# fenghansen/YOND_public

Measured on AMD Instinct MI355X. Metric: Bayer megapixels/sec end-to-end (NLE+VST+denoise+iVST), higher is better.
Workload: dtype f32 (3x3 convolutions: f32 operands as two f16 halves -- 22-23 significant bits -- on the f16 MFMA, 3 products per f32 product, f32 accumulate; per-layer error vs float64 asserted <= 2x the f32 direct kernel's and <= 2e-5 of max|ref| (tests/test_hip_conv.py; measured 1.3e-6 vs 1.5e-6), whole frame v

## Files before the change

### yond_public_amd/csrc/conv_s2_tall.hip

```cpp
#include "common.h"

typedef _Float16 f16x8 __attribute__((ext_vector_type(8)));
typedef _Float16 f16x4 __attribute__((ext_vector_type(4)));
#define S2T_GLOBAL __attribute__((address_space(1)))

namespace {
constexpr int S2T_TH = 8;
constexpr int S2T_IH = (S2T_TH - 1) * 2 + 3;
constexpr int S2T_IW = 31 * 2 + 3;
constexpr int S2T_HALF = (S2T_IW + 1) / 2;
constexpr int S2T_TWP = 2 * S2T_HALF;
constexpr int S2T_PLANE = S2T_IH * S2T_TWP * 4;
constexpr int S2T_IMG = 4 * S2T_PLANE + 4;
constexpr int S2T_W = 9 * 2 * 2 * 64 * 4;
constexpr int S2T_NWV = S2T_W / 4;
constexpr int S2T_NWT = (S2T_NWV + 511) / 512;
constexpr int S2T_NITEM = S2T_IH * S2T_IW * 4;
constexpr int S2T_NIN = (S2T_NITEM + 511) / 512;
constexpr int S2T_FILM = 1536;
constexpr int S2T_W_OFF = S2T_IMG, S2T_FILM_OFF = S2T_W_OFF + 2 * S2T_W;
constexpr int S2T_SMEM = (S2T_FILM_OFF + 2 * S2T_FILM) * 4;
static_assert(S2T_SMEM <= 160 * 1024, "LDS budget");
static_assert((S2T_NIN - 1) * 512 < S2T_NITEM, "only a thread's last item may lie past the tile");

__device__ __forceinline__ float s2t_silu(float x) {
    return x * __builtin_amdgcn_rcpf(1.0f + __builtin_amdgcn_exp2f(x * -1.44269504088896341f));
}
}

template <bool D2>
__global__ __launch_bounds__(512) void conv_s2_tall_kernel(const YondConvDesc d) {
    extern __shared__ __attribute__((aligned(16))) float smem[];
    const int tid = threadIdx.x, lane = tid & 63, wave = __builtin_amdgcn_readfirstlane(tid >> 6);
    const int li = lane & 31, lh = lane >> 5;
    const int rg = wave & 3, cg = wave >> 2;
    const int nct = d.Cout / 64, ntx = (d.Wo + 31) / 32, nty = (d.Ho + S2T_TH - 1) / S2T_TH;
    const int total = nct * ntx * nty * d.N;
    const int G = gridDim.x;
    const int lslot = (G % 8 == 0) ? (blockIdx.x % 8) * (G / 8) + blockIdx.x / 8 : blockIdx.x;
    const int nchunk = d.C0 / 16;
    const bool rev = d.tile_order != 0;
    const int PS0 = YOND_SP_PLANE_UNITS(d.H, d.W);
    if (lslot >= total) return;
    const bool clk_on = d.clk != nullptr && blockIdx.x == 0 && tid == 0;
    unsigned long long clk_c0 = 0, clk_r0 = 0;
    if (clk_on) { clk_c0 = __builtin_amdgcn_s_memtime(); clk_r0 = __builtin_amdgcn_s_memrealtime(); }
    asm volatile("" : "+v"(clk_c0), "+v"(clk_r0));
    float* dst_v = d.dst;
    char* dst2_v = (char*)d.dst2;
    unsigned int* word_v = d.status;
    unsigned long long* clk_v = d.clk;
    asm volatile("" : "+v"(dst_v), "+v"(dst2_v), "+v"(word_v), "+v"(clk_v));
    int nct_v = nct, ntx_v = ntx, nty_v = nty;
    unsigned ps2_v = (unsigned)YOND_SP_PLANE_UNITS(d.Ho, d.Wo);
    asm volatile("" : "+v"(nct_v), "+v"(ntx_v), "+v"(nty_v), "+v"(ps2_v));

    {
        const int nf = (d.ebatch ? d.N : 1) * d.Cout;
        for (int i = tid; i < nf; i += 512) {
            smem[S2T_FILM_OFF + i] = d.escale ? d.escale[i] : 1.0f;
            smem[S2T_FILM_OFF + S2T_FILM + i] = d.eshift ? d.eshift[i] : 0.0f;
        }
    }

    int in_lds[S2T_NIN];
#pragma unroll
    for (int k = 0; k < S2T_NIN; ++k) {
        const int it = tid + k * 512;
        const int pix = it >> 2, py = pix / S2T_IW, px = pix % S2T_IW;
        const int lp = py * S2T_TWP + (px & 1) * S2T_HALF + (px >> 1);
        in_lds[k] = it < S2T_NITEM ? (it & 3) * S2T_PLANE + lp * 4 : 4 * S2T_PLANE;
    }

    struct Tile { int ct, n, ox0, oy0; };
    auto origin = [&](int t) {
        Tile T;
        int b = t;
        T.ct = b % nct_v; b /= nct_v;
        const int tx = b % ntx_v; b /= ntx_v;
        const int ty = b % nty_v, n = b / nty_v;
        T.n = __builtin_amdgcn_readfirstlane(rev ? d.N - 1 - n : n);
        T.ct = __builtin_amdgcn_readfirstlane(T.ct);
        T.ox0 = __builtin_amdgcn_readfirstlane((rev ? ntx_v - 1 - tx : tx) * 32);
        T.oy0 = __builtin_amdgcn_readfirstlane((rev ? nty_v - 1 - ty : ty) * S2T_TH);
        return T;
    };
    unsigned voff[S2T_NIN];
    auto decode = [&](const Tile& T) {
#pragma unroll
        for (int k = 0; k < S2T_NIN; ++k) {
            const int it = tid + k * 512;
            const int pix = it >> 2, py = pix / S2T_IW, px = pix % S2T_IW;
            const int gy = T.oy0 * 2 - 1 + py, gx = T.ox0 * 2 - 1 + px;
            const bool in = it < S2T_NITEM && gy >= 0 && gy < d.H && gx >= 0 && gx < d.W;
            voff[k] = ((unsigned)(it & 3) * (unsigned)PS0 + (unsigned)(in ? gy * d.W + gx : d.H * d.W)) * 16u;
        }
    };
    auto uniform_ptr = [&](const void* p) {
        const unsigned long long a = (unsigned long long)(uintptr_t)p;
        const unsigned lo = __builtin_amdgcn_readfirstlane((unsigned)a), hi = __builtin_amdgcn_readfirstlane((unsigned)(a >> 32));
        return (const char*)(uintptr_t)(((unsigned long long)hi << 32) | lo);
    };
    auto in_base = [&](const Tile& T, int ch) { return (const char*)d.src0 + (size_t)(T.n * nchunk + ch) * 4 * (size_t)PS0 * 16; };
    auto w_base = [&](const Tile& T, int ch) { return uniform_ptr(d.wpk + ((size_t)T.ct * nchunk + ch) * S2T_W); };
    f32x4 vin[S2T_NIN];
    auto issue_load = [&](auto kc, const char* ib) __attribute__((always_inline)) {
        constexpr int k = decltype(kc)::value;
        vin[k] = *(const S2T_GLOBAL f32x4*)(const S2T_GLOBAL char*)(ib + voff[k]);
    };
    auto issue_dma = [&](auto kc, const char* wsrc, float* wbuf) __attribute__((always_inline)) {
        constexpr int k = decltype(kc)::value;
        const unsigned lds0 = (unsigned)(uintptr_t)(__attribute__((address_space(3))) float*)wbuf;
        const int it = tid + k * 512;
        const int it_wave = __builtin_amdgcn_readfirstlane(it - lane);
        const unsigned lds_wave = __builtin_amdgcn_readfirstlane(lds0 + (unsigned)it_wave * 16u);
        const unsigned vo = (unsigned)it * 16u;
        if ((k + 1) * 512 <= S2T_NWV || it_wave < S2T_NWV)
            asm volatile("s_mov_b32 m0, %0\n\ts_nop 0\n\tglobal_load_lds_dwordx4 %1, %2" ::"s"(lds_wave), "v"(vo), "s"(wsrc) : "memory");
    };
    auto write_in = [&]() __attribute__((always_inline)) {
#pragma unroll
        for (int k = 0; k < S2T_NIN; ++k) *(f32x4*)(smem + in_lds[k]) = vin[k];
    };

    f32x16 acc[2][2];
    auto zero_acc = [&]() {
#pragma unroll
        for (int a = 0; a < 2; ++a)
#pragma unroll
            for (int m = 0; m < 2; ++m)
#pragma unroll
                for (int r = 0; r < 16; ++r) acc[a][m][r] = 0.0f;
    };

    const int x_off = (lh * 2) * S2T_PLANE + ((rg * 4) * S2T_TWP + li) * 4;
    const int w_off = ((lh * 2) * 64 + cg * 32 + li) * 4;
    const bool wave_hi = wave >= 4;
    const char* ib_s = nullptr;
    const char* wsrc_s = nullptr;
    auto mfma_step = [&](const float* wcur, float* wnext, auto&& prep) __attribute__((always_inline)) {
        typedef const __attribute__((address_space(3))) f16x8* lds_h8;
        const __attribute__((address_space(3))) float* xb = (const __attribute__((address_space(3))) float*)(smem + x_off);
        const __attribute__((address_space(3))) float* wb = (const __attribute__((address_space(3))) float*)(wcur + w_off);
        constexpr int R = 5, NQ = 3 * R, XD = 3, Q0 = 2, NQW = NQ - Q0, NOPS = S2T_NWT + S2T_NIN;
        f16x8 xr[XD][2], wt[2][3][2];
        auto loadX = [&](auto qc) __attribute__((always_inline)) {
            constexpr int q = decltype(qc)::value, dx = q / R, r = q % R;
            constexpr int xo = (dx & 1) * S2T_HALF + (dx >> 1);
#pragma unroll
            for (int p = 0; p < 2; ++p) xr[q % XD][p] = *(lds_h8)(xb + p * S2T_PLANE + (r * S2T_TWP + xo) * 4);
        };
        auto loadW = [&](auto dc) __attribute__((always_inline)) {
            constexpr int dx = decltype(dc)::value;
#pragma unroll
            for (int dy = 0; dy < 3; ++dy)
#pragma unroll
                for (int p = 0; p < 2; ++p) wt[dx % 2][dy][p] = *(lds_h8)(wb + (((dy * 3 + dx) * 4 + p) * 64) * 4);
        };
        loadW(IntC<0>{});
        loadX(IntC<0>{});
        loadX(IntC<1>{});
        static_for<0, NQ>([&](auto qc) __attribute__((always_inline)) {
            constexpr int q = decltype(qc)::value, dx = q / R, r = q % R;
            constexpr bool wpre = r == 2 && dx < 2;
            if constexpr (q + 2 < NQ) loadX(IntC<q + 2>{});
            if constexpr (wpre) loadW(IntC<dx + 1>{});
            constexpr int nmf = 3 * ((r <= 2 ? 1 : 0) + (r >= 2 ? 1 : 0));
#pragma unroll
            for (int a = 0; a < 3; ++a) {
#pragma unroll
                for (int m = 0; m < 2; ++m) {
                    const int dy = r - 2 * m;
                    if (dy < 0 || dy > 2) continue;
                    acc[a == 1 ? 0 : 1][m] = __builtin_amdgcn_mfma_f32_32x32x16_f16(wt[dx % 2][dy][a == 2 ? 1 : 0], xr[q % XD][a == 0 ? 1 : 0],
                                                                                    acc[a == 1 ? 0 : 1][m], 0, 0, 0);
                }
            }
            if constexpr (q == 0) { if (wave_hi) __builtin_amdgcn_s_setprio(1); }
            if constexpr (q == NQ / 2) { if (wave_hi) __builtin_amdgcn_s_setprio(0); }
            if constexpr (q == Q0 - 1) prep();
            constexpr int qq = q >= Q0 ? q - Q0 : 0;
            constexpr int o_lo = q >= Q0 ? (qq * NOPS + NQW - 1) / NQW : 0, o_hi = q >= Q0 ? ((qq + 1) * NOPS + NQW - 1) / NQW : 0;
            static_for<o_lo, (o_hi < NOPS ? o_hi : NOPS)>([&](auto oc) __attribute__((always_inline)) {
                constexpr int o = decltype(oc)::value;
                if constexpr (o < S2T_NWT) issue_dma(IntC<o>{}, wsrc_s, wnext);
                else issue_load(IntC<o - S2T_NWT>{}, ib_s);
            });
            constexpr int nrd = (q + 2 < NQ ? 2 : 0) + (wpre ? 6 : 0);
            constexpr int l_lo = o_lo > S2T_NWT ? o_lo : S2T_NWT, nld = o_hi > l_lo ? o_hi - l_lo : 0;
            if constexpr (nrd > 0) __builtin_amdgcn_sched_group_barrier(0x100, nrd, 0);
#pragma unroll
            for (int i = 0; i < nmf; ++i) {
                __builtin_amdgcn_sched_group_barrier(0x008, 1, 0);
                if (i == 0 && nld > 0) __builtin_amdgcn_sched_group_barrier(0x020, nld, 0);
            }
        });
    };

    float slope_eff = d.post_act == 2 ? d.slope : 1.0f;
    asm volatile("" : "+v"(slope_eff));
    YondRange amax;
    auto epilogue = [&](const Tile& T) __attribute__((always_inline)) {
        const int ox = T.ox0 + li;
        const bool col_ok = ox < d.Wo;
        const int cbase = T.ct * 64 + cg * 32 + 4 * lh;
        const float* fs = smem + S2T_FILM_OFF + (d.ebatch ? T.n * d.Cout : 0) + cbase;
        const long long hw = (long long)d.Ho * d.Wo;
        f32x4 es[4], et[4];
#pragma unroll
        for (int g = 0; g < 4; ++g) {
            es[g] = *(const f32x4*)(fs + 8 * g);
            et[g] = *(const f32x4*)(fs + S2T_FILM + 8 * g);
        }
#pragma unroll
        for (int m = 0; m < 2; ++m) {
            const int oy = T.oy0 + rg * 2 + m;
            const bool ok = col_ok && oy < d.Ho;
            const long long pixo = (long long)oy * d.Wo + ox;
            float* op = dst_v + (((long long)T.n * (d.Cout / 4) + cbase / 4) * hw + pixo) * 4;
            const long long gstep = 8LL * hw;
#pragma unroll
            for (int g = 0; g < 4; ++g) {
                f32x4 v;
#pragma unroll
                for (int e = 0; e < 4; ++e) {
                    float x = acc[0][m][4 * g + e];
                    x = fmaf(acc[1][m][4 * g + e], 1.0f / 2048.0f, x);
                    x = fmaf(x, es[g][e], et[g][e]);
                    x = x > 0.0f ? x : x * slope_eff;
                    v[e] = x + 0.0f;
                }
                if (ok) *(S2T_GLOBAL f32x4*)(S2T_GLOBAL float*)(op + g * gstep) = v;
                if constexpr (D2) {
                    f32x4 a;
#pragma unroll
                    for (int e = 0; e < 4; ++e) a[e] = s2t_silu(v[e]);
                    amax.add(a);
                    const f16x4 h = {(_Float16)a[0], (_Float16)a[1], (_Float16)a[2], (_Float16)a[3]};
                    const int c8 = cbase - 4 * lh + 8 * g;
                    const size_t PS2 = (size_t)ps2_v;
                    char* pp = dst2_v + ((size_t)(((T.n * (d.Cout / 16) + (c8 >> 4)) * 2 + ((c8 >> 3) & 1)) * 2) * PS2 + (size_t)pixo) * 16 + lh * 8;
                    if (ok) *(S2T_GLOBAL f16x4*)(S2T_GLOBAL char*)pp = h;
                    const f16x4 l = {(_Float16)((a[0] - (float)h[0]) * 2048.0f), (_Float16)((a[1] - (float)h[1]) * 2048.0f),
                                     (_Float16)((a[2] - (float)h[2]) * 2048.0f), (_Float16)((a[3] - (float)h[3]) * 2048.0f)};
                    if (ok) *(S2T_GLOBAL f16x4*)(S2T_GLOBAL char*)(pp + PS2 * 16) = l;
                }
            }
        }
    };

    struct Cur { int tile, ch; };
    auto adv = [&](Cur c) {
        Cur n;
        const bool last = c.ch + 1 == nchunk;
        n.tile = last ? c.tile + G : c.tile;
        n.ch = last ? 0 : c.ch + 1;
        return n;
    };
    Cur cs = {lslot, 0};
    Tile lt = origin(lslot), cur = lt;
    auto park = [&](Tile& T) { asm volatile("" : "+v"(T.ct), "+v"(T.n), "+v"(T.ox0), "+v"(T.oy0)); };
    park(cur);
    float* w0 = smem + S2T_W_OFF;
    float* w1 = w0 + S2T_W;
    decode(lt);
    {
        const char* ws = w_base(lt, 0);
        const char* ib = in_base(lt, 0);
        static_for<0, S2T_NWT>([&](auto kc) __attribute__((always_inline)) { issue_dma(kc, ws, w0); });
        static_for<0, S2T_NIN>([&](auto kc) __attribute__((always_inline)) { issue_load(kc, ib); });
    }
    zero_acc();
    asm volatile("s_waitcnt vmcnt(0)" ::: "memory");
    write_in();
    asm volatile("s_waitcnt vmcnt(0) lgkmcnt(0)\n\ts_barrier" ::: "memory");
    while (true) {
        const bool last_ch = cs.ch + 1 == nchunk;
        const Cur cn = adv(cs);
        auto prep = [&]() __attribute__((always_inline)) {
            if (last_ch && cn.tile < total) {
                lt = origin(cn.tile);
                decode(lt);
            }
            ib_s = in_base(lt, cn.ch);
            wsrc_s = w_base(lt, cn.ch);
        };
        mfma_step(w0, w1, prep);
        asm volatile("s_waitcnt lgkmcnt(0)\n\ts_barrier" ::: "memory");
        asm volatile("s_waitcnt vmcnt(0)" ::: "memory");
        write_in();
        if (last_ch) {
            epilogue(cur);
            zero_acc();
            cur = lt;
            park(cur);
        }
        asm volatile("s_waitcnt lgkmcnt(0)\n\ts_barrier" ::: "memory");
        if (cn.tile >= total) break;
        cs = cn;
        float* t = w0;
        w0 = w1;
        w1 = t;
    }
    if constexpr (D2) {
        if (word_v && !amax.at_most(65504.0f)) atomicOr(word_v, YOND_STATUS_HALF_OVERFLOW);
    }
    if (clk_on) {
        atomicAdd(clk_v, __builtin_amdgcn_s_memtime() - clk_c0);
        atomicAdd(clk_v + 1, __builtin_amdgcn_s_memrealtime() - clk_r0);
    }
}

static bool s2t_takes(const YondConvDesc& d) {
    if (d.ksize != 3 || d.stride != 2 || d.shuffle != 0 || d.tn != 64 || !d.src0 || d.src1 || d.C1 != 0 || !d.dst || !d.wpk) return false;
    if (d.in_fmt != YOND_FMT_SPLIT_PLANES || d.out_fmt != YOND_FMT_PLANES4 || d.res_fmt || d.res || d.out4_dst || d.pre_act) return false;
    if (d.post_act != 0 && d.post_act != 2) return false;
    if (d.N <= 0 || d.H <= 0 || d.W <= 0 || d.Ho != (d.H + 1) / 2 || d.Wo != (d.W + 1) / 2) return false;
    if (d.C0 <= 0 || d.C0 % 16 || d.Cout <= 0 || d.Cout % 64) return false;
    if ((long long)(d.ebatch ? d.N : 1) * d.Cout > S2T_FILM) return false;
    if ((long long)d.N * d.H * d.W > 0x7fffffffLL) return false;
    if ((long long)d.N * (d.C0 / 16) * 4 * YOND_SP_PLANE_UNITS(d.H, d.W) * 4 >= 0x7fffffffLL) return false;
    if ((long long)YOND_SP_PLANE_UNITS(d.H, d.W) * 16 * 4 >= 0x7fffffffLL) return false;
    const long long tiles = (long long)(d.Cout / 64) * ((d.Wo + 31) / 32) * ((d.Ho + S2T_TH - 1) / S2T_TH) * d.N;
    if (tiles > 0x7fffffffLL) return false;
    if (d.Wo <= 16) {
        const int f = d.Wo <= 8 ? 4 : 2;
        const long long subs = (long long)d.N * ((d.Ho + 3) / 4) * ((d.Wo + 32 / f - 1) / (32 / f));
        const long long tiles_f = (long long)(d.Cout / 64) * ((subs + f - 1) / f), tiles4 = (long long)(d.Cout / 64) * ((d.Ho + 3) / 4) * d.N;
        const bool fits = (long long)d.H * d.W * d.C0 * 4 * f < (1LL << 31);
        if (fits && (tiles_f + 255) / 256 < (tiles4 + 255) / 256) return false;
    }
    return true;
}

extern "C" int yond_conv_s2_tall_supported(const YondConvDesc* d) { return (d && (d->algo == 3 || d->algo == 7) && s2t_takes(*d)) ? 1 : 0; }

template <bool D2>
static int launch_s2t(const YondConvDesc& d, hipStream_t st) {
    static bool attr_set = false;
    auto kern = conv_s2_tall_kernel<D2>;
    if (!attr_set) {
        hipError_t e = hipFuncSetAttribute((const void*)kern, hipFuncAttributeMaxDynamicSharedMemorySize, S2T_SMEM);
        if (e != hipSuccess) return (int)e;
        attr_set = true;
    }
    const long long total = (long long)(d.Cout / 64) * ((d.Wo + 31) / 32) * ((d.Ho + S2T_TH - 1) / S2T_TH) * d.N;
    const int grid = total < 256 ? (int)total : 256;
    hipLaunchKernelGGL(kern, dim3(grid), dim3(512), S2T_SMEM, st, d);
    YOND_LAUNCH_CHECK();
    return YOND_OK;
}

int yond_conv_s2_tall_dispatch(const YondConvDesc& d, hipStream_t st) {
    if (!s2t_takes(d)) return YOND_EUNSUPPORTED;
    return d.dst2 ? launch_s2t<true>(d, st) : launch_s2t<false>(d, st);
}
```

### yond_public_amd/engine.py

```python
import ctypes as C
import os

import numpy as np
import torch

from . import _lib as L


def _rup(c, m=32):
    return (c + m - 1) // m * m


def _np_ptr(a):
    return C.c_void_p(a.ctypes.data)


FILM_MAX_C = 1024


WINO_DEFAULT = 'split'


SPLIT_PLANES = True
SP_FLOW = True
HALF_FLOW = True
HALF_K1_TN128 = True
HALF_S2_TN128 = True
HALF_FLOW_TN128 = True
HALF_TN128 = True
FUSE_OUT4 = True
FUSE_BLOCK0 = False
K1_SUB2 = True
K1_D2_LEVELS = (3,)
K1_STATIONARY_LEVELS = (2, 1, 0)
S2_TALL_LEVELS = (0, 1, 2)
K1_D2_LEVELS_HALF = ()
SP_CONV1_MIN_LEVEL = 3
UNET_SP = True
SNAKE_ORDER = True


def sp_plane_units(H, W):
    return (H * W + 8) // 8 * 8


class _PackedConv:

    def __init__(self, dev, weight, bias, ksize, stride, splits, shuffle=False):
        lib = L.load()
        w = weight.detach().to('cpu', torch.float32).numpy()
        if shuffle:
            cin, cout = w.shape[0], w.shape[1]
            coutp = _rup(cout)
            m = np.zeros((4, coutp, cin), np.float32)
            m[:, :cout, :] = w.transpose(2, 3, 1, 0).reshape(4, cout, cin)
            w = m.reshape(4 * coutp, cin, 1, 1)
            self.cout_real_p = coutp
            gemm_n = 4 * coutp
        else:
            cout = w.shape[0]
            coutp = _rup(cout)
            gemm_n = coutp
            self.cout_real_p = coutp
        assert sum(splits) == w.shape[1], (splits, w.shape)
        psplits = [_rup(s) for s in splits]
        cinp = sum(psplits)
        wp = np.zeros((gemm_n, cinp, ksize, ksize), np.float32)
        so, do = 0, 0
        for s, ps in zip(splits, psplits):
            wp[:w.shape[0], do:do + s] = w[:, so:so + s]
            so += s
            do += ps
        self._wp = np.ascontiguousarray(wp)
        self._packed = {}
        self._dev = dev
        b = torch.zeros(coutp, dtype=torch.float32)
        if bias is not None:
            b[:cout] = bias.detach().to('cpu', torch.float32)
        self.bias = b.to(dev)
        self.ksize, self.stride, self.shuffle = ksize, stride, shuffle
        self.psplits, self.gemm_n, self.coutp, self.cinp = psplits, gemm_n, coutp, cinp
        self.cin_real, self.cout_real = sum(splits), cout
        self.config(0, 0, 0)
        self.wmax = float(np.abs(self._wp).max()) if self._wp.size else 0.0
        self.macs_per_pixel = self.cin_real * self.cout_real * (4 if shuffle else ksize * ksize)

    def config(self, N, Ho, Wo, split=False):
        lib = L.load()
        tn, kc = C.c_int(), C.c_int()
        L.check(lib.yond_conv_config(self.ksize, self.stride, self.cinp, self.gemm_n, int(self.shuffle), N, Ho, Wo,
                                     C.byref(tn), C.byref(kc)), "yond_conv_config")
        key = (tn.value, kc.value, bool(split))
        if key not in self._packed:
            packed = np.empty(self._wp.size, np.float32)
            fn = lib.yond_pack_conv_weight_split_f32 if split else lib.yond_pack_conv_weight_f32
            rc = fn(_np_ptr(self._wp), self.gemm_n, self.cinp, self.ksize, tn.value, kc.value, _np_ptr(packed))
            if split and rc == -2:
                self._packed[key] = None
            else:
                L.check(rc, "yond_pack_conv_weight_f32")
                self._packed[key] = torch.from_numpy(packed).to(self._dev)
        return tn.value, kc.value, self._packed[key]

    def wino(self):
        lib = L.load()
        if self.ksize != 3 or self.stride != 1 or self.shuffle:
            return None
        tn = int(lib.yond_conv_wino_supported(self.cinp, self.gemm_n))
        if not tn:
            return None
        if 'wino' not in self._packed:
            packed = np.empty(16 * self.gemm_n * self.cinp, np.float32)
            L.check(lib.yond_pack_conv_wino_weight_f32(_np_ptr(self._wp), self.gemm_n, self.cinp, tn, _np_ptr(packed)),
                    "yond_pack_conv_wino_weight_f32")
            self._packed['wino'] = (tn, torch.from_numpy(packed).to(self._dev))
        return self._packed['wino']

    def split(self, parts=2, wide=True, wide_s2=False):
        lib = L.load()
        if self.shuffle != (self.ksize == 1):
            return None
        tn = int(lib.yond_conv_split_supported(self.ksize, self.stride, self.cinp, self.gemm_n))
        if not tn:
            return None
        if parts == 1 and wide and HALF_TN128 and tn == 64 and self.ksize == 3 and self.stride == 1 and self.gemm_n % 128 == 0:
            tn = 128
        if parts == 1 and wide_s2 and tn == 64 and self.ksize == 3 and self.stride == 2 and self.gemm_n % 128 == 0:
            tn = 128
        if parts == 1 and wide_s2 and tn == 64 and self.ksize == 1 and self.shuffle == 1 and (self.gemm_n // 4) % 128 == 0:
            tn = 128
        key = ('split', parts) if tn != 128 else ('split', parts, 128)
        if key not in self._packed:
            packed = np.empty(self._wp.size * parts // 2, np.float32)
            rc = lib.yond_pack_conv_split_weight_f32(_np_ptr(self._wp), self.gemm_n, self.cinp, self.ksize, tn, parts, _np_ptr(packed))
            if rc == -2:
                self._packed[key] = None
                return None
            L.check(rc, "yond_pack_conv_split_weight_f32")
            self._packed[key] = (tn, torch.from_numpy(packed).to(self._dev))
        return self._packed[key]


class _PackedUpSub2:

    def __init__(self, dev, w_f, b_f, c):
        lib = L.load()
        assert c % 32 == 0 and w_f.shape == (3 * c, c, 2, 2)
        w = w_f.detach().to('cpu', torch.float32).numpy()
        k = (4 * c + 47) // 48 * 48
        m = np.zeros((2, c // 32, 2, 32, k), np.float32)
        for dy in range(2):
            for dx in range(2):
                wc = w[:2 * c, :, dy, dx].T.reshape(c // 32, 32, 2 * c)
                ws = w[2 * c:, :, dy, dx].T.reshape(c // 32, 32, c)
                m[dy, :, dx, :, :2 * c] = wc
                m[dy, :, dx, :, 2 * c + dx * c:2 * c + (dx + 1) * c] = ws
        self._wp = np.ascontiguousarray(m.reshape(4 * c, k, 1, 1))
        self._dev, self._wpk = dev, {}
        self.ok = self._pack(2) is not None
        b = torch.zeros(c, dtype=torch.float32)
        b[:] = b_f.detach().to('cpu', torch.float32)
        self.bias = b.to(dev)
        self.psplits, self.gemm_n, self.coutp, self.cinp = [2 * c, k - 2 * c], 4 * c, c, k
        self.ksize, self.stride, self.shuffle = 1, 1, 2
        self.cout_real_p = c
        self.wmax = float(np.abs(self._wp).max())
        self.macs_per_pixel = 2 * c * c * 4 + 2 * c * c * 4

    def _pack(self, parts):
        if parts not in self._wpk:
            packed = np.empty(self._wp.size * parts // 2, np.float32)
            rc = L.load().yond_pack_conv_split_weight_f32(_np_ptr(self._wp), self._wp.shape[0], self._wp.shape[1], 1, 64, parts, _np_ptr(packed))
            self._wpk[parts] = torch.from_numpy(packed).to(self._dev) if rc == 0 else None
        return self._wpk[parts]

    def split(self, parts=2, wide=True, wide_s2=False):
        return (64, self._pack(parts)) if (self.ok and self._pack(parts) is not None) else None

    def wino(self):
        return None


class DenoiserPlan:

    def __init__(self, module, device):
        self._init_launcher(device, getattr(module, 'precision', 'fp32'))
        self.kind = type(module).__name__
        self.res = bool(module.res)
        self.norm = bool(module.norm)
        sd = {k: v.detach() for k, v in module.state_dict().items()}
        self.sd = sd
        self.guided = self.kind in ('GuidedResUnet', 'SNRnet')
        dev = self.dev
        if self.guided:
            nf = sd['conv_in.weight'].shape[0]
            self.nf = nf
            self.conv_in_w, self.conv_in_b = self._pack_conv_in(sd['conv_in.weight'], sd['conv_in.bias'])
            self.blocks = {}
            chans = [nf, nf * 2, nf * 4, nf * 8, nf * 16, nf * 8, nf * 4, nf * 2, nf]
            film = []
            for i, c in enumerate(chans, start=1):
                pre = f'conv{i}'
                blk = {'C': c, 'Cp': _rup(c)}
                blk['conv1'] = _PackedConv(dev, sd[pre + '.conv1.weight'], None, 3, 1, [c])
                blk['conv2'] = _PackedConv(dev, sd[pre + '.conv2.weight'], None, 3, 1, [c])
                if i >= 6:
                    wt = sd[f'upv{i}.weight'].to('cpu', torch.float64)
                    bt = sd[f'upv{i}.bias'].to('cpu', torch.float64)
                    wsc = sd[pre + '.short_cut.0.weight'].to('cpu', torch.float64)[:, :, 0, 0]
                    bsc = sd[pre + '.short_cut.0.bias'].to('cpu', torch.float64)
                    w_cur = torch.einsum('ou,iuyx->ioyx', wsc[:, :c], wt)
                    w_skip = wsc[:, c:].t()[:, :, None, None].expand(c, c, 2, 2)
                    w_f = torch.cat([w_cur, w_skip], 0).to(torch.float32).contiguous()
                    b_f = (bsc + wsc[:, :c] @ bt).to(torch.float32)
                    blk['upsc'] = _PackedConv(dev, w_f, b_f, 1, 1, [2 * c, c], shuffle=True)
                    blk['upsc'].macs_per_pixel = 2 * c * c * 4 + 2 * c * c * 4
                    if c == 32:
                        up2 = _PackedUpSub2(dev, w_f, b_f, c)
                        if up2.ok:
                            blk['upsc2'] = up2
                if i <= 4:
                    blk['pool'] = _PackedConv(dev, sd[f'pool{i}.conv.weight'], sd[f'pool{i}.conv.bias'], 3, 2, [c])
                self.blocks[i] = blk
                film.append((pre, c))
            self._film_spec = film
            self._film_cache = {}
            self.w_out = self._pad_out_w(sd['conv10.weight'])
            self.b_out = sd['conv10.bias'].to(dev, torch.float32).contiguous()
            self._film_params = {k: v.to(dev, torch.float32).contiguous() for k, v in sd.items()
                                 if any(s in k for s in ('.gamma.', '.beta.', '.sfm1.', '.sfm2.', '.conv1.bias', '.conv2.bias'))}
        else:
            nf = sd['conv1_1.weight'].shape[0]
            self.nf = nf
            self.conv_in_w, self.conv_in_b = self._pack_conv_in(sd['conv1_1.weight'], sd['conv1_1.bias'])
            self.convs = {}
            c = nf
            self.convs['conv1_2'] = _PackedConv(dev, sd['conv1_2.weight'], sd['conv1_2.bias'], 3, 1, [c])
            for i in range(2, 6):
                self.convs[f'conv{i}_1'] = _PackedConv(dev, sd[f'conv{i}_1.weight'], sd[f'conv{i}_1.bias'], 3, 1, [c])
                c *= 2
                self.convs[f'conv{i}_2'] = _PackedConv(dev, sd[f'conv{i}_2.weight'], sd[f'conv{i}_2.bias'], 3, 1, [c])
            for i in range(6, 10):
                self.convs[f'upv{i}'] = _PackedConv(dev, sd[f'upv{i}.weight'], sd[f'upv{i}.bias'], 1, 1, [c], shuffle=True)
                c //= 2
                self.convs[f'conv{i}_1'] = _PackedConv(dev, sd[f'conv{i}_1.weight'], sd[f'conv{i}_1.bias'], 3, 1, [c, c])
                self.convs[f'conv{i}_2'] = _PackedConv(dev, sd[f'conv{i}_2.weight'], sd[f'conv{i}_2.bias'], 3, 1, [c])
            self.w_out = self._pad_out_w(sd['conv10_1.weight'])
            self.b_out = sd['conv10_1.bias'].to(dev, torch.float32).contiguous()

    def _init_launcher(self, device, precision):
        self.lib = L.load()
        self.dev = torch.device(device)
        self.prof = None
        self.status = torch.zeros(12, dtype=torch.int32, device=self.dev)
        self.status_slot = 0
        self.strict = False
        self.precision = precision

    def _pack_conv_in(self, w, b):
        w = w.detach().to('cpu', torch.float32).numpy()
        cout = w.shape[0]
        if w.shape[1] != 4:
            raise L.YondHipError(f"first layer must have 4 input channels (packed Bayer), got {w.shape[1]}")
        coutp = _rup(cout)
        wp = np.zeros((coutp, 4, 3, 3), np.float32)
        wp[:cout] = w
        packed = np.empty(coutp * 40, np.float32)
        L.check(self.lib.yond_pack_conv_in_weight_f32(_np_ptr(wp), coutp, _np_ptr(packed)), "yond_pack_conv_in_weight_f32")
        bp = torch.zeros(coutp, dtype=torch.float32)
        bp[:cout] = b.detach().to('cpu', torch.float32)
        return torch.from_numpy(packed).to(self.dev), bp.to(self.dev)

    def _pad_out_w(self, w):
        w = w.detach().to('cpu', torch.float32).reshape(w.shape[0], -1)
        if w.shape[0] != 4:
            raise L.YondHipError(f"last layer must have 4 output channels, got {w.shape[0]}")
        wp = torch.zeros(4, _rup(w.shape[1]), dtype=torch.float32)
        wp[:, :w.shape[1]] = w
        return wp.to(self.dev).contiguous()

    def _split_pair(self, pc1, pc2):
        if getattr(self, 'strict', False) or getattr(self, 'conv_algo', WINO_DEFAULT) != 'split':
            return False
        prec = getattr(self, 'precision', 'fp32')
        if prec not in ('fp32', 'fp16'):
            return False
        parts = 2 if prec == 'fp32' else 1
        return all(pc.ksize == 3 and pc.stride == 1 and pc.split(parts) is not None for pc in (pc1, pc2))

    def _sp_flow(self, N, H, W):
        if not (SPLIT_PLANES and SP_FLOW) or getattr(self, 'strict', False) or getattr(self, 'conv_algo', WINO_DEFAULT) != 'split':
            return False
        prec = getattr(self, 'precision', 'fp32')
        if prec not in ('fp32', 'fp16') or (prec == 'fp16' and not HALF_FLOW) or sp_plane_units(H, W) * 64 * 4 >= 2 ** 31:
            return False
        parts = 2 if prec == 'fp32' else 1
        for i, blk in self.blocks.items():
            for k in ('conv1', 'conv2', 'pool', 'upsc'):
                if k in blk and blk[k].split(parts, wide=False) is None:
                    return False
        return self._out4_fusable(self.blocks[9]['conv2'], flow=True)

    def _out4_fusable(self, pc, flow=False):
        prec = getattr(self, 'precision', 'fp32')
        return (not getattr(self, 'strict', False) and getattr(self, 'conv_algo', WINO_DEFAULT) == 'split' and (prec == 'fp32' or (prec == 'fp16' and flow))
                and pc.ksize == 3 and pc.stride == 1 and pc.gemm_n == 32 and pc.split(2 if prec == 'fp32' else 1) is not None and FUSE_OUT4)

    def _new_sp(self, key, N, H, W, Cc, parts=2):
        cache = self.__dict__.setdefault('_sp_cache', {})
        k = (key, N, H, W, Cc, parts, getattr(self, 'lane', 0))
        if k not in cache:
            cache[k] = torch.zeros(N * (Cc // 16) * 2 * parts * sp_plane_units(H, W) * 4, dtype=torch.float32, device=self.dev)
        return cache[k]

    def _conv(self, pc, src0, src1, N, H, W, dst, escale=None, eshift=None, ebatch=0, res=None, pre_act=0, post_act=0,
              slope=0.0, algo=None, out4=None, in_fmt=0, out_fmt=0, res_fmt=0, dst2=None, stationary=False, s2_tall=False):
        d = L.YondConvDesc()
        d.src0 = src0.data_ptr()
        d.src1 = src1.data_ptr() if src1 is not None else None
        d.C0 = pc.psplits[0]
        d.C1 = pc.psplits[1] if len(pc.psplits) > 1 else 0
        d.N, d.H, d.W = N, H, W
        if pc.stride == 2:
            d.Ho, d.Wo = (H + 1) // 2, (W + 1) // 2
        else:
            d.Ho, d.Wo = H, W
        d.Cout = pc.gemm_n
        d.ksize, d.stride, d.shuffle = pc.ksize, pc.stride, int(pc.shuffle)
        d.pre_act, d.post_act, d.slope = pre_act, post_act, slope
        prec = getattr(self, 'precision', 'fp32')
        if getattr(self, 'strict', False) and algo is None:
            prec, algo = 'fp32-mfma', 1
        if algo is None:
            algo = getattr(self, 'conv_algo', WINO_DEFAULT)
            if prec == 'fp32-mfma' and algo == 'split':
                algo = 1
            if prec == 'fp16' and WINO_DEFAULT == 'split':
                algo = 'half'
# ... 352 lines not shown
```

Measured before the change: 2713.

## Add register-resident-weight s2 tall conv form with double-buffered input DMA

Adds a second form of the stride-2 tall conv kernel. It keeps the 3x3 weights in registers, loaded straight from global memory, and streams the input tile into double-buffered LDS with global_load_lds DMA instead of staging it through registers. This form is used whenever C0 != 32, and the tall kernel is also enabled for level 3. The intent is to remove the register-to-LDS input write and the barrier it needs, and to overlap input fetch with the MFMAs. In exchange it uses more VGPRs for the weights and does per-chunk global weight reloads.

```diff
diff --git a/yond_public_amd/csrc/conv_s2_tall.hip b/yond_public_amd/csrc/conv_s2_tall.hip
--- a/yond_public_amd/csrc/conv_s2_tall.hip
+++ b/yond_public_amd/csrc/conv_s2_tall.hip
@@ -22,15 +22,21 @@
 constexpr int S2T_SMEM = (S2T_FILM_OFF + 2 * S2T_FILM) * 4;
 static_assert(S2T_SMEM <= 160 * 1024, "LDS budget");
 static_assert((S2T_NIN - 1) * 512 < S2T_NITEM, "only a thread's last item may lie past the tile");
-
+constexpr int S2T2_NDMA = (4 * S2T_IH * S2T_TWP + 511) / 512;
+constexpr int S2T2_IMG = S2T2_NDMA * 512 * 4;
+constexpr int S2T2_FILM_OFF = 2 * S2T2_IMG;
+constexpr int S2T2_SMEM = (S2T2_FILM_OFF + 2 * S2T_FILM) * 4;
+static_assert(S2T2_SMEM <= 160 * 1024, "LDS budget");
+static_assert(S2T2_NDMA == S2T_NIN, "both forms keep one offset per thread and instruction");
 __device__ __forceinline__ float s2t_silu(float x) {
     return x * __builtin_amdgcn_rcpf(1.0f + __builtin_amdgcn_exp2f(x * -1.44269504088896341f));
 }
 }
 
-template <bool D2>
-__global__ __launch_bounds__(512) void conv_s2_tall_kernel(const YondConvDesc d) {
+template <bool D2, bool TWO>
+__device__ __forceinline__ void s2t_body(const YondConvDesc& d) {
     extern __shared__ __attribute__((aligned(16))) float smem[];
+    constexpr int FILM_OFF = TWO ? S2T2_FILM_OFF : S2T_FILM_OFF;
     const int tid = threadIdx.x, lane = tid & 63, wave = __builtin_amdgcn_readfirstlane(tid >> 6);
     const int li = lane & 31, lh = lane >> 5;
     const int rg = wave & 3, cg = wave >> 2;
@@ -58,18 +64,20 @@
     {
         const int nf = (d.ebatch ? d.N : 1) * d.Cout;
         for (int i = tid; i < nf; i += 512) {
-            smem[S2T_FILM_OFF + i] = d.escale ? d.escale[i] : 1.0f;
-            smem[S2T_FILM_OFF + S2T_FILM + i] = d.eshift ? d.eshift[i] : 0.0f;
-        }
-    }
-
-    int in_lds[S2T_NIN];
-#pragma unroll
-    for (int k = 0; k < S2T_NIN; ++k) {
-        const int it = tid + k * 512;
-        const int pix = it >> 2, py = pix / S2T_IW, px = pix % S2T_IW;
-        const int lp = py * S2T_TWP + (px & 1) * S2T_HALF + (px >> 1);
-        in_lds[k] = it < S2T_NITEM ? (it & 3) * S2T_PLANE + lp * 4 : 4 * S2T_PLANE;
+            smem[FILM_OFF + i] = d.escale ? d.escale[i] : 1.0f;
+            smem[FILM_OFF + S2T_FILM + i] = d.eshift ? d.eshift[i] : 0.0f;
+        }
+    }
+
+    int in_lds[TWO ? 1 : S2T_NIN];
+    if constexpr (!TWO) {
+#pragma unroll
+        for (int k = 0; k < S2T_NIN; ++k) {
+            const int it = tid + k * 512;
+            const int pix = it >> 2, py = pix / S2T_IW, px = pix % S2T_IW;
+            const int lp = py * S2T_TWP + (px & 1) * S2T_HALF + (px >> 1);
+            in_lds[k] = it < S2T_NITEM ? (it & 3) * S2T_PLANE + lp * 4 : 4 * S2T_PLANE;
+        }
     }
 
     struct Tile { int ct, n, ox0, oy0; };
@@ -89,11 +97,20 @@
     auto decode = [&](const Tile& T) {
 #pragma unroll
         for (int k = 0; k < S2T_NIN; ++k) {
-            const int it = tid + k * 512;
-            const int pix = it >> 2, py = pix / S2T_IW, px = pix % S2T_IW;
-            const int gy = T.oy0 * 2 - 1 + py, gx = T.ox0 * 2 - 1 + px;
-            const bool in = it < S2T_NITEM && gy >= 0 && gy < d.H && gx >= 0 && gx < d.W;
-            voff[k] = ((unsigned)(it & 3) * (unsigned)PS0 + (unsigned)(in ? gy * d.W + gx : d.H * d.W)) * 16u;
+            if constexpr (TWO) {
+                const int u = tid + k * 512;
+                const int pl = u / (S2T_IH * S2T_TWP), rem = u - pl * (S2T_IH * S2T_TWP);
+                const int py = rem / S2T_TWP, c = rem - py * S2T_TWP, hf = c >= S2T_HALF ? 1 : 0, px = 2 * (c - hf * S2T_HALF) + hf;
+                const int gy = T.oy0 * 2 - 1 + py, gx = T.ox0 * 2 - 1 + px;
+                const bool in = pl < 4 && px < S2T_IW && gy >= 0 && gy < d.H && gx >= 0 && gx < d.W;
+                voff[k] = ((unsigned)(pl & 3) * (unsigned)PS0 + (unsigned)(in ? gy * d.W + gx : d.H * d.W)) * 16u;
+            } else {
+                const int it = tid + k * 512;
+                const int pix = it >> 2, py = pix / S2T_IW, px = pix % S2T_IW;
+                const int gy = T.oy0 * 2 - 1 + py, gx = T.ox0 * 2 - 1 + px;
+                const bool in = it < S2T_NITEM && gy >= 0 && gy < d.H && gx >= 0 && gx < d.W;
+                voff[k] = ((unsigned)(it & 3) * (unsigned)PS0 + (unsigned)(in ? gy * d.W + gx : d.H * d.W)) * 16u;
+            }
         }
     };
     auto uniform_ptr = [&](const void* p) {
@@ -103,7 +120,7 @@
     };
     auto in_base = [&](const Tile& T, int ch) { return (const char*)d.src0 + (size_t)(T.n * nchunk + ch) * 4 * (size_t)PS0 * 16; };
     auto w_base = [&](const Tile& T, int ch) { return uniform_ptr(d.wpk + ((size_t)T.ct * nchunk + ch) * S2T_W); };
-    f32x4 vin[S2T_NIN];
+    f32x4 vin[TWO ? 1 : S2T_NIN];
     auto issue_load = [&](auto kc, const char* ib) __attribute__((always_inline)) {
         constexpr int k = decltype(kc)::value;
         vin[k] = *(const S2T_GLOBAL f32x4*)(const S2T_GLOBAL char*)(ib + voff[k]);
@@ -119,8 +136,25 @@
             asm volatile("s_mov_b32 m0, %0\n\ts_nop 0\n\tglobal_load_lds_dwordx4 %1, %2" ::"s"(lds_wave), "v"(vo), "s"(wsrc) : "memory");
     };
     auto write_in = [&]() __attribute__((always_inline)) {
-#pragma unroll
-        for (int k = 0; k < S2T_NIN; ++k) *(f32x4*)(smem + in_lds[k]) = vin[k];
+        if constexpr (!TWO) {
+#pragma unroll
+            for (int k = 0; k < S2T_NIN; ++k) *(f32x4*)(smem + in_lds[k]) = vin[k];
+        }
+    };
+    auto issue_in_dma = [&](auto kc, const char* ib, float* img) __attribute__((always_inline)) {
+        constexpr int k = decltype(kc)::value;
+        const unsigned lds0 = (unsigned)(uintptr_t)(__attribute__((address_space(3))) float*)img;
+        const unsigned lds_wave = __builtin_amdgcn_readfirstlane(lds0 + (unsigned)((k * 8 + wave) * 1024));
+        const unsigned vo = voff[k];
+        asm volatile("s_mov_b32 m0, %0\n\ts_nop 0\n\tglobal_load_lds_dwordx4 %1, %2" ::"s"(lds_wave), "v"(vo), "s"(ib) : "memory");
+    };
+    f16x8 wr[3][3][2];
+    const unsigned w_goff = (unsigned)((((lane >> 5) * 2) * 64 + (wave >> 2) * 32 + (lane & 31)) * 16);
+    auto load_wr = [&](auto dc, auto yc, const char* ws) __attribute__((always_inline)) {
+        constexpr int dx = decltype(dc)::value, dy = decltype(yc)::value;
+#pragma unroll
+        for (int p = 0; p < 2; ++p)
+            wr[dx][dy][p] = *(const S2T_GLOBAL f16x8*)(const S2T_GLOBAL char*)(ws + w_goff + (unsigned)((((dy * 3 + dx) * 4 + p) * 64) * 16));
     };
 
     f32x16 acc[2][2];
@@ -197,6 +231,52 @@
         });
     };
 
+    constexpr int S2T2_QE = 10;
+    constexpr int S2T2_AFTER = 2 * (5 - ((S2T2_QE - 1) % 5 > 2 ? (S2T2_QE - 1) % 5 : 2) + 3 * (2 - (S2T2_QE - 1) / 5));
+    static_assert(S2T2_QE > 2 && S2T2_QE <= 15, "the DMAs sit in groups Q0 .. QE - 1");
+    auto mfma_step2 = [&](const float* img, float* inext, auto&& prep) __attribute__((always_inline)) {
+        typedef const __attribute__((address_space(3))) f16x8* lds_h8;
+        const __attribute__((address_space(3))) float* xb = (const __attribute__((address_space(3))) float*)(img + x_off);
+        constexpr int R = 5, NQ = 3 * R, XD = 3, Q0 = 2, NQW = S2T2_QE - Q0, NOPS = S2T2_NDMA;
+        f16x8 xr[XD][2];
+        auto loadX = [&](auto qc) __attribute__((always_inline)) {
+            constexpr int q = decltype(qc)::value, dx = q / R, r = q % R;
+            constexpr int xo = (dx & 1) * S2T_HALF + (dx >> 1);
+#pragma unroll
+            for (int p = 0; p < 2; ++p) xr[q % XD][p] = *(lds_h8)(xb + p * S2T_PLANE + (r * S2T_TWP + xo) * 4);
+        };
+        loadX(IntC<0>{});
+        loadX(IntC<1>{});
+        static_for<0, NQ>([&](auto qc) __attribute__((always_inline)) {
+            constexpr int q = decltype(qc)::value, dx = q / R, r = q % R;
+            constexpr bool wrep = r >= 2;
+            if constexpr (q + 2 < NQ) loadX(IntC<q + 2>{});
+            constexpr int nmf = 3 * ((r <= 2 ? 1 : 0) + (r >= 2 ? 1 : 0));
+#pragma unroll
+            for (int a = 0; a < 3; ++a) {
+#pragma unroll
+                for (int m = 0; m < 2; ++m) {
+                    const int dy = r - 2 * m;
+                    if (dy < 0 || dy > 2) continue;
+                    acc[a == 1 ? 0 : 1][m] = __builtin_amdgcn_mfma_f32_32x32x16_f16(wr[dx][dy][a == 2 ? 1 : 0], xr[q % XD][a == 0 ? 1 : 0],
+                                                                                    acc[a == 1 ? 0 : 1][m], 0, 0, 0);
+                }
+            }
+            if constexpr (q == 0) { if (wave_hi) __builtin_amdgcn_s_setprio(1); }
+            if constexpr (q == NQ / 2) { if (wave_hi) __builtin_amdgcn_s_setprio(0); }
+            if constexpr (q == Q0 - 1) prep();
+            constexpr bool dq = q >= Q0 && q < S2T2_QE;
+            constexpr int qq = dq ? q - Q0 : 0;
+            constexpr int o_lo = dq ? (qq * NOPS + NQW - 1) / NQW : 0, o_hi = dq ? ((qq + 1) * NOPS + NQW - 1) / NQW : 0;
+            static_for<o_lo, (o_hi < NOPS ? o_hi : NOPS)>([&](auto oc) __attribute__((always_inline)) { issue_in_dma(oc, ib_s, inext); });
+            if constexpr (wrep) load_wr(IntC<dx>{}, IntC<r - 2>{}, wsrc_s);
+            if constexpr (q + 2 < NQ) __builtin_amdgcn_sched_group_barrier(0x100, 2, 0);
+#pragma unroll
+            for (int i = 0; i < nmf; ++i) __builtin_amdgcn_sched_group_barrier(0x008, 1, 0);
+            if constexpr (wrep) __builtin_amdgcn_sched_group_barrier(0x020, 2, 0);
+        });
+    };
+
     float slope_eff = d.post_act == 2 ? d.slope : 1.0f;
     asm volatile("" : "+v"(slope_eff));
     YondRange amax;
@@ -204,7 +284,7 @@
         const int ox = T.ox0 + li;
         const bool col_ok = ox < d.Wo;
         const int cbase = T.ct * 64 + cg * 32 + 4 * lh;
-        const float* fs = smem + S2T_FILM_OFF + (d.ebatch ? T.n * d.Cout : 0) + cbase;
+        const float* fs = smem + FILM_OFF + (d.ebatch ? T.n * d.Cout : 0) + cbase;
         const long long hw = (long long)d.Ho * d.Wo;
         f32x4 es[4], et[4];
 #pragma unroll
@@ -261,46 +341,90 @@
     Tile lt = origin(lslot), cur = lt;
     auto park = [&](Tile& T) { asm volatile("" : "+v"(T.ct), "+v"(T.n), "+v"(T.ox0), "+v"(T.oy0)); };
     park(cur);
-    float* w0 = smem + S2T_W_OFF;
-    float* w1 = w0 + S2T_W;
-    decode(lt);
-    {
-        const char* ws = w_base(lt, 0);
-        const char* ib = in_base(lt, 0);
-        static_for<0, S2T_NWT>([&](auto kc) __attribute__((always_inline)) { issue_dma(kc, ws, w0); });
-        static_for<0, S2T_NIN>([&](auto kc) __attribute__((always_inline)) { issue_load(kc, ib); });
-    }
-    zero_acc();
-    asm volatile("s_waitcnt vmcnt(0)" ::: "memory");
-    write_in();
-    asm volatile("s_waitcnt vmcnt(0) lgkmcnt(0)\n\ts_barrier" ::: "memory");
-    while (true) {
-        const bool last_ch = cs.ch + 1 == nchunk;
-        const Cur cn = adv(cs);
-        auto prep = [&]() __attribute__((always_inline)) {
-            if (last_ch && cn.tile < total) {
-                lt = origin(cn.tile);
-                decode(lt);
-            }
-            ib_s = in_base(lt, cn.ch);
-            wsrc_s = w_base(lt, cn.ch);
-        };
-        mfma_step(w0, w1, prep);
-        asm volatile("s_waitcnt lgkmcnt(0)\n\ts_barrier" ::: "memory");
+    if constexpr (TWO) {
+        float* i0 = smem;
+        float* i1 = smem + S2T2_IMG;
+        decode(lt);
+        {
+            const char* ws = w_base(lt, 0);
+            const char* ib = uniform_ptr(in_base(lt, 0));
+            static_for<0, 3>([&](auto dc) __attribute__((always_inline)) {
+                static_for<0, 3>([&](auto yc) __attribute__((always_inline)) { load_wr(dc, yc, ws); });
+            });
+            static_for<0, S2T2_NDMA>([&](auto kc) __attribute__((always_inline)) { issue_in_dma(kc, ib, i0); });
+        }
+        zero_acc();
+        asm volatile("s_waitcnt vmcnt(0) lgkmcnt(0)\n\ts_barrier" ::: "memory");
+#pragma unroll
+        for (int i = 0; i < 18; ++i) asm volatile("" : "+v"(wr[i / 6][(i / 2) % 3][i % 2]));
+        while (true) {
+            const bool last_ch = cs.ch + 1 == nchunk;
+            const Cur cn = adv(cs);
+            auto prep = [&]() __attribute__((always_inline)) {
+                if (last_ch && cn.tile < total) {
+                    lt = origin(cn.tile);
+                    decode(lt);
+                }
+                ib_s = uniform_ptr(in_base(lt, cn.ch));
+                wsrc_s = w_base(lt, cn.ch);
+            };
+            mfma_step2(i0, i1, prep);
+            asm volatile("s_waitcnt vmcnt(%0)" ::"n"(S2T2_AFTER) : "memory");
+            if (last_ch) {
+                epilogue(cur);
+                zero_acc();
+                cur = lt;
+                park(cur);
+            }
+            asm volatile("s_waitcnt lgkmcnt(0)\n\ts_barrier" ::: "memory");
+            if (cn.tile >= total) break;
+            cs = cn;
+            float* t = i0;
+            i0 = i1;
+            i1 = t;
+        }
+    } else {
+        float* w0 = smem + S2T_W_OFF;
+        float* w1 = w0 + S2T_W;
+        decode(lt);
+        {
+            const char* ws = w_base(lt, 0);
+            const char* ib = in_base(lt, 0);
+            static_for<0, S2T_NWT>([&](auto kc) __attribute__((always_inline)) { issue_dma(kc, ws, w0); });
+            static_for<0, S2T_NIN>([&](auto kc) __attribute__((always_inline)) { issue_load(kc, ib); });
+        }
+        zero_acc();
         asm volatile("s_waitcnt vmcnt(0)" ::: "memory");
         write_in();
-        if (last_ch) {
-            epilogue(cur);
-            zero_acc();
-            cur = lt;
-            park(cur);
-        }
-        asm volatile("s_waitcnt lgkmcnt(0)\n\ts_barrier" ::: "memory");
-        if (cn.tile >= total) break;
-        cs = cn;
-        float* t = w0;
-        w0 = w1;
-        w1 = t;
+        asm volatile("s_waitcnt vmcnt(0) lgkmcnt(0)\n\ts_barrier" ::: "memory");
+        while (true) {
+            const bool last_ch = cs.ch + 1 == nchunk;
+            const Cur cn = adv(cs);
+            auto prep = [&]() __attribute__((always_inline)) {
+                if (last_ch && cn.tile < total) {
+                    lt = origin(cn.tile);
+                    decode(lt);
+                }
+                ib_s = in_base(lt, cn.ch);
+                wsrc_s = w_base(lt, cn.ch);
+            };
+            mfma_step(w0, w1, prep);
+            asm volatile("s_waitcnt lgkmcnt(0)\n\ts_barrier" ::: "memory");
+            asm volatile("s_waitcnt vmcnt(0)" ::: "memory");
+            write_in();
+            if (last_ch) {
+                epilogue(cur);
+                zero_acc();
+                cur = lt;
+                park(cur);
+            }
+            asm volatile("s_waitcnt lgkmcnt(0)\n\ts_barrier" ::: "memory");
+            if (cn.tile >= total) break;
+            cs = cn;
+            float* t = w0;
+            w0 = w1;
+            w1 = t;
+        }
     }
     if constexpr (D2) {
         if (word_v && !amax.at_most(65504.0f)) atomicOr(word_v, YOND_STATUS_HALF_OVERFLOW);
@@ -309,6 +433,15 @@
         atomicAdd(clk_v, __builtin_amdgcn_s_memtime() - clk_c0);
         atomicAdd(clk_v + 1, __builtin_amdgcn_s_memrealtime() - clk_r0);
     }
+}
+
+template <bool D2>
+__global__ __launch_bounds__(512) void conv_s2_tall_kernel(const YondConvDesc d) {
+    s2t_body<D2, true>(d);
+}
+template <bool D2>
+__global__ __launch_bounds__(512) void conv_s2_tall_kernel_one_image(const YondConvDesc d) {
+    s2t_body<D2, false>(d);
 }
 
 static bool s2t_takes(const YondConvDesc& d) {
@@ -335,23 +468,30 @@
 
 extern "C" int yond_conv_s2_tall_supported(const YondConvDesc* d) { return (d && (d->algo == 3 || d->algo == 7) && s2t_takes(*d)) ? 1 : 0; }
 
-template <bool D2>
+template <bool D2, bool TWO>
 static int launch_s2t(const YondConvDesc& d, hipStream_t st) {
     static bool attr_set = false;
-    auto kern = conv_s2_tall_kernel<D2>;
+    constexpr int SMEM = TWO ? S2T2_SMEM : S2T_SMEM;
+    auto kern = TWO ? conv_s2_tall_kernel<D2> : conv_s2_tall_kernel_one_image<D2>;
     if (!attr_set) {
-        hipError_t e = hipFuncSetAttribute((const void*)kern, hipFuncAttributeMaxDynamicSharedMemorySize, S2T_SMEM);
+        hipError_t e = hipFuncSetAttribute((const void*)kern, hipFuncAttributeMaxDynamicSharedMemorySize, SMEM);
         if (e != hipSuccess) return (int)e;
         attr_set = true;
     }
     const long long total = (long long)(d.Cout / 64) * ((d.Wo + 31) / 32) * ((d.Ho + S2T_TH - 1) / S2T_TH) * d.N;
     const int grid = total < 256 ? (int)total : 256;
-    hipLaunchKernelGGL(kern, dim3(grid), dim3(512), S2T_SMEM, st, d);
+    hipLaunchKernelGGL(kern, dim3(grid), dim3(512), SMEM, st, d);
     YOND_LAUNCH_CHECK();
     return YOND_OK;
 }
 
 int yond_conv_s2_tall_dispatch(const YondConvDesc& d, hipStream_t st) {
     if (!s2t_takes(d)) return YOND_EUNSUPPORTED;
-    return d.dst2 ? launch_s2t<true>(d, st) : launch_s2t<false>(d, st);
-}
+    bool two = d.C0 != 32;
+#ifdef YOND_EXPERIMENTS
+    const long form = yond_exp_long("YOND_S2T_FORM", 0);
+    if (form == 1 || form == 2) two = form == 2;
+#endif
+    if (two) return d.dst2 ? launch_s2t<true, true>(d, st) : launch_s2t<false, true>(d, st);
+    return d.dst2 ? launch_s2t<true, false>(d, st) : launch_s2t<false, false>(d, st);
+}
diff --git a/yond_public_amd/engine.py b/yond_public_amd/engine.py
--- a/yond_public_amd/engine.py
+++ b/yond_public_amd/engine.py
@@ -33,7 +33,7 @@
 K1_SUB2 = True
 K1_D2_LEVELS = (3,)
 K1_STATIONARY_LEVELS = (2, 1, 0)
-S2_TALL_LEVELS = (0, 1, 2)
+S2_TALL_LEVELS = (0, 1, 2, 3)
 K1_D2_LEVELS_HALF = ()
 SP_CONV1_MIN_LEVEL = 3
 UNET_SP = True
```

New measurement: 2744 (median of 6 runs). +1.1%, better.
